# stardist/stardist

Measured on AMD Instinct MI355X. Metric: predict_instances() Mpix/s (2D) + Mvox/s (3D) end-to-end at 1/2/4/8 GPU, higher is better.
Workload: dtype f32

## Files before the change

### stardist_amd/csrc/nms2d.hip

```cpp
#include <type_traits>

#include "common.h"
#include "clip_sweep.h"
#include "clip_beam.h"
#include "area_bounds.h"
#include "poly_pass.h"
#include "nms_rounds.h"
#include "../../include/stardist_hip.h"
#include <hipcub/hipcub.hpp>
#include <math.h>
#include <stdlib.h>
#include <vector>

namespace {

using sdclip::i64;

__device__ __forceinline__ float wave_min(float v) { for (int o = 32; o; o >>= 1) v = fminf(v, __shfl_xor(v, o)); return v; }
__device__ __forceinline__ float wave_max(float v) { for (int o = 32; o; o >>= 1) v = fmaxf(v, __shfl_xor(v, o)); return v; }
__device__ __forceinline__ i64 wave_sum(i64 v) { for (int o = 32; o; o >>= 1) v += __shfl_xor(v, o); return v; }

__global__ void __launch_bounds__(256) k_build(const float* __restrict__ dist, const float* __restrict__ pts,
                                               const float2* __restrict__ sincos, int N, int R,
                                               int* __restrict__ vx, int* __restrict__ vy, int4* __restrict__ bbox,
// ... 67 lines not shown
  if (c < R) ssc[c] = sincos[c];
  {
    const int* g = (const int*)dist + (size_t)base * R;
    const int nv = vec4 ? nel >> 2 : 0;
    for (int e = c; e < nv; e += 64) ((int4*)rows)[e] = ((const int4*)g)[e];
    for (int e = 4 * nv + c; e < nel; e += 64) rows[e] = g[e];
  }
  __syncthreads();
  const bool cv = c < cnt;
  float rmax = 0.f;
  int iy = INT32_MAX, ix = INT32_MAX, iyh = INT32_MIN, ixh = INT32_MIN;
  if (cv) {
    const int i = base + c;
    const float py = pts[2 * i], px = pts[2 * i + 1];
    float xmin = INFINITY, xmax = -INFINITY, ymin = INFINITY, ymax = -INFINITY;
    i64 s = 0, sa = 0;
    int X0 = 0, Y0 = 0, Xp = 0, Yp = 0;
    int k = c % R;
    for (int t = 0; t < R; ++t) {
      const float d = __int_as_float(rows[c * R + k]);
      const float2 sc = ssc[k];
      const float y = py + d * sc.x;
      const float x = px + d * sc.y;
      xmin = fminf(xmin, x); xmax = fmaxf(xmax, x);
      ymin = fminf(ymin, y); ymax = fmaxf(ymax, y);
      rmax = fmaxf(rmax, d);
      const int X = (int)(long long)x, Y = (int)(long long)y;
      sx[c * R + k] = X; sy[c * R + k] = Y;
      if (t) { const i64 cr = (i64)Xp * Y - (i64)Yp * X; s += cr; sa += (cr < 0 ? -cr : cr); }
      else { X0 = X; Y0 = Y; }
      Xp = X; Yp = Y;
      k = (k + 1 == R) ? 0 : k + 1;
    }
    { const i64 cr = (i64)Xp * Y0 - (i64)Yp * X0; s += cr; sa += (cr < 0 ? -cr : cr); }
    float a;
    if (sa < (1ll << 24)) a = (float)s;
    else {
      a = 0.f;
      for (int q = 0; q < R; ++q) {
        const int qn = (q + 1 == R) ? 0 : q + 1;
        a += (float)((i64)sx[c * R + q] * sy[c * R + qn] - (i64)sy[c * R + q] * sx[c * R + qn]);
      }
    }
    area[i] = (float)(0.5 * (double)fabsf(a));
    radius[i] = rmax;
    bbox[i] = make_int4((int)xmin, (int)xmax, (int)ymin, (int)ymax);
    iy = iyh = (int)floorf(py); ix = ixh = (int)floorf(px);
  }
  for (int o = 32; o; o >>= 1) {
    rmax = fmaxf(rmax, __shfl_xor(rmax, o));
    iy = min(iy, __shfl_xor(iy, o)); iyh = max(iyh, __shfl_xor(iyh, o));
    ix = min(ix, __shfl_xor(ix, o)); ixh = max(ixh, __shfl_xor(ixh, o));
  }
  if (c == 0) {
    const int rb = __float_as_int(rmax);
    volatile int* gs = gstats;
    if (rb > gs[0]) atomicMax(&gstats[0], rb);
    if (iy < gs[1]) atomicMin(&gstats[1], iy);
    if (iyh > gs[2]) atomicMax(&gstats[2], iyh);
    if (ix < gs[3]) atomicMin(&gstats[3], ix);
    if (ixh > gs[4]) atomicMax(&gstats[4], ixh);
  }
  __syncthreads();
  {
    int* gx = vx + (size_t)base * R;
    int* gy = vy + (size_t)base * R;
    const int nv = vec4 ? nel >> 2 : 0;
    for (int e = c; e < nv; e += 64) { ((int4*)gx)[e] = ((const int4*)sx)[e]; ((int4*)gy)[e] = ((const int4*)sy)[e]; }
    for (int e = 4 * nv + c; e < nel; e += 64) { gx[e] = sx[e]; gy[e] = sy[e]; }
  }
}

struct GridP { float y0, x0, inv_cs; int ny, nx; };

__device__ __forceinline__ int cell_of(const GridP g, float py, float px, int& cy, int& cx) {
  cy = (int)((py - g.y0) * g.inv_cs); cx = (int)((px - g.x0) * g.inv_cs);
  cy = min(max(cy, 0), g.ny - 1); cx = min(max(cx, 0), g.nx - 1);
  return cy * g.nx + cx;
}

struct Window { int ylo, yhi, xlo, xhi; };
__device__ __forceinline__ Window cell_window(const GridP g, bool by_bbox, float reach, const int4 bb, float py, float px) {
  float y0, y1, x0, x1;
  if (by_bbox) { x0 = (float)bb.x - reach; x1 = (float)bb.y + reach; y0 = (float)bb.z - reach; y1 = (float)bb.w + reach; }
  else { const float rr = 2.f * reach; x0 = px - rr; x1 = px + rr; y0 = py - rr; y1 = py + rr; }
  Window w;
  w.ylo = min(max((int)floorf((y0 - 0.5f - g.y0) * g.inv_cs), 0), g.ny - 1); w.yhi = min(max((int)floorf((y1 + 0.5f - g.y0) * g.inv_cs), 0), g.ny - 1);
  w.xlo = min(max((int)floorf((x0 - 0.5f - g.x0) * g.inv_cs), 0), g.nx - 1); w.xhi = min(max((int)floorf((x1 + 0.5f - g.x0) * g.inv_cs), 0), g.nx - 1);
  return w;
}
constexpr int MAX_WIN_ROWS = 32;

__global__ void k_cell_count(const float* __restrict__ pts, int N, GridP g, int* __restrict__ cellCount, int* __restrict__ candCell) {
  const int i = blockIdx.x * blockDim.x + threadIdx.x;
  if (i >= N) return;
  int cy, cx;
  const int c = cell_of(g, pts[2 * i], pts[2 * i + 1], cy, cx);
  candCell[i] = c;
  atomicAdd(&cellCount[c], 1);
}
struct __attribute__((aligned(16))) CellRec { int4 bb; float py, px, area; int j; };
__global__ void k_cell_fill(int N, const int* __restrict__ candCell, const int* __restrict__ cellStart,
                            int* __restrict__ cellFill, const float* __restrict__ pts, const int4* __restrict__ bbox,
                            const float* __restrict__ area, CellRec* __restrict__ rec, GridP g, int by_bbox, float reach, int* __restrict__ slotCap) {
  const int i = blockIdx.x * blockDim.x + threadIdx.x;
  if (i >= N) return;
  const int c = candCell[i];
  const int pos = atomicAdd(&cellFill[c], 1);
  CellRec r;
  r.bb = bbox[i]; r.py = pts[2 * i]; r.px = pts[2 * i + 1]; r.area = area[i]; r.j = i;
  rec[cellStart[c] + pos] = r;
  if (slotCap) {
    const Window w = cell_window(g, by_bbox != 0, reach, r.bb, r.py, r.px);
    int u = -1;
    for (int yy = w.ylo; yy <= w.yhi; ++yy) u += cellStart[yy * g.nx + w.xhi + 1] - cellStart[yy * g.nx + w.xlo];
    slotCap[i] = u;
    if (i == 0) slotCap[N] = 0;
  }
}

__device__ __forceinline__ bool bbox_intersect(const int4 a, const int4 b) {
  return (b.x <= a.y && a.x <= b.y && b.z <= a.w && a.z <= b.w);
}

__device__ __forceinline__ bool may_interact(const NmsFlags f, const int4 bi, const int4 bj, float pyi, float pxi, float pyj, float pxj,
                                             float ai, float aj) {
  if (f.thr_nonneg) {
    if (!bbox_intersect(bi, bj)) return false;
    const float wh = (float)(min(bi.y, bj.y) - max(bi.x, bj.x)) * (float)(min(bi.w, bj.w) - max(bi.z, bj.z));
    return wh * 1.00001f >= f.thr * fminf(ai, aj) * 0.99999f;
  }
  bool ok = true;
  if (f.use_bbox) ok = ok && bbox_intersect(bi, bj);
  if (f.use_kdtree) {
    const float dy = pyi - pyj, dxx = pxi - pxj;
    const float rr = 2.f * f.max_dist + 1.f;
    ok = ok && (dy * dy + dxx * dxx < rr * rr);
  }
  return ok;
}

struct WindowRuns { int rbeg, excl, nrows, total; };
__device__ __forceinline__ WindowRuns window_runs(const GridP g, const Window win, const int* __restrict__ cellStart, int lane) {
  WindowRuns w;
  w.nrows = __builtin_amdgcn_readfirstlane(win.yhi - win.ylo + 1);
  int rbeg = 0, rlen = 0;
  if (lane < w.nrows) { rbeg = cellStart[(win.ylo + lane) * g.nx + win.xlo]; rlen = cellStart[(win.ylo + lane) * g.nx + win.xhi + 1] - rbeg; }
  int incl = rlen;
  for (int o = 1; o < MAX_WIN_ROWS; o <<= 1) { const int t = __shfl_up(incl, o); if (lane >= o) incl += t; }
  w.total = __builtin_amdgcn_readlane(incl, w.nrows - 1);
  w.rbeg = rbeg; w.excl = incl - rlen;
  return w;
}
template <class Body>
__device__ __forceinline__ void walk_window(const WindowRuns& w, int lane, Body&& body) {
  int r0 = 0;
  for (int t = 0; t < w.total; t += 64) {
    while (r0 + 1 < w.nrows && __builtin_amdgcn_readlane(w.excl, r0 + 1) <= t) ++r0;
    int rb = __builtin_amdgcn_readlane(w.rbeg, r0), re = __builtin_amdgcn_readlane(w.excl, r0);
    const int v = t + lane;
    for (int r = r0 + 1; r < w.nrows; ++r) {
      const int e_r = __builtin_amdgcn_readlane(w.excl, r);
      if (e_r > t + 63) break;
      const int b_r = __builtin_amdgcn_readlane(w.rbeg, r);
      if (e_r <= v) { rb = b_r; re = e_r; }
    }
    body(v < w.total ? rb + (v - re) : -1);
  }
}

template <int MODE>
__global__ void __launch_bounds__(256) k_neighbours(int N, GridP g, NmsFlags f, const CellRec* __restrict__ rec, const int* __restrict__ cellStart,
                                                    int* __restrict__ nbrCount, int* __restrict__ nbrLow, const i64* __restrict__ nbrStart,
                                                    int* __restrict__ nbr, int* __restrict__ waitOn, int by_bbox, float reach) {
  const int wave = threadIdx.x >> 6, lane = threadIdx.x & 63;
  const int per = gridDim.x >> 3;
  const int blk = (blockIdx.x & 7) * per + (blockIdx.x >> 3);
  const int w = blk * (blockDim.x >> 6) + wave;
  if (w >= N) return;
  const CellRec me = rec[w];
  const int i = me.j;
  const int4 bi = me.bb;
  const float pyi = me.py, pxi = me.px, ai = me.area;
  int nLo = 0;
  int minj = INT32_MAX;
  const i64 base = MODE ? nbrStart[i] : 0;
  const WindowRuns runs = window_runs(g, cell_window(g, by_bbox != 0, reach, bi, pyi, pxi), cellStart, lane);
  walk_window(runs, lane, [&](int ri) {
    bool hit = false;
    int j = -1;
    if (ri >= 0) {
      const CellRec r = rec[ri];
      j = r.j;
      if (j < i) hit = may_interact(f, bi, r.bb, pyi, pxi, r.py, r.px, ai, r.area);
    }
    const unsigned long long m = __ballot(hit);
    if (MODE && hit) { nbr[base + nLo + __popcll(m & ((1ull << lane) - 1))] = j; if (j < minj) minj = j; }
    nLo += __popcll(m);
  });
  if (!MODE && lane == 0) nbrCount[i] = nLo;
  if (MODE != 1 && lane == 0) nbrLow[i] = nLo;
  if (MODE) {
    for (int o = 32; o; o >>= 1) minj = min(minj, __shfl_xor(minj, o));
    if (lane == 0) waitOn[i] = (minj < i) ? minj : WAIT_NONE;
  }
}

constexpr int EMIT_STAGE = 512;
__global__ void __launch_bounds__(256) k_round_emit(const int* __restrict__ K, const int* __restrict__ nKPtr, unsigned char* __restrict__ state,
                                                    GridP g, const CellRec* __restrict__ rec, const int* __restrict__ cellStart, int by_bbox, float reach,
                                                    NmsFlags f, const float* __restrict__ pts, const int4* __restrict__ bbox,
                                                    const float* __restrict__ radius, const float* __restrict__ area,
                                                    int2* __restrict__ pairs, unsigned long long* pairCount,
                                                    unsigned long long pairCap) {
  const int wave = threadIdx.x >> 6, lane = threadIdx.x & 63;
  const int nK = *nKPtr;
  __shared__ int2 stage[4][EMIT_STAGE];
  int nst = 0;
  auto flush = [&]() {
    if (!nst) return;
    unsigned long long base = 0;
    if (lane == 0) base = atomicAdd(pairCount, (unsigned long long)nst);
    base = __shfl(base, 0);
    __builtin_amdgcn_wave_barrier();
    for (int k = lane; k < nst; k += 64) { const unsigned long long pos = base + k; if (pos < pairCap) pairs[pos] = stage[wave][k]; }
    __builtin_amdgcn_wave_barrier();
    nst = 0;
  };
  for (int w = blockIdx.x * (blockDim.x >> 6) + wave; w < nK; w += gridDim.x * (blockDim.x >> 6)) {
    const int i = K[w];
    if (lane == 0) state[i] = ST_KEPT;
    const int4 bi = bbox[i];
    const float pyi = pts[2 * i], pxi = pts[2 * i + 1];
    const double ai = (double)area[i] + 1.e-10;
    const float rad = f.max_dist + radius[i];
    const float rad2 = rad * rad;
    const WindowRuns runs = window_runs(g, cell_window(g, by_bbox != 0, reach, bi, pyi, pxi), cellStart, lane);
    walk_window(runs, lane, [&](int ri) {
      bool emit = false;
      int j = -1;
      if (ri >= 0) {
        const CellRec r = rec[ri];
        j = r.j;
        bool ok = j > i;
        if (ok && f.use_kdtree) {
          const float d0 = pyi - r.py, d1 = pxi - r.px;
          float d2 = d0 * d0; d2 += d1 * d1;
          ok = d2 < rad2;
        }
        if (ok && (f.use_bbox || f.thr_nonneg)) {
          const int4 bj = r.bb;
          ok = bbox_intersect(bi, bj);
          if (ok && f.thr_nonneg) {
            const double w = (double)(min(bi.y, bj.y) - max(bi.x, bj.x)), hgt = (double)(min(bi.w, bj.w) - max(bi.z, bj.z));
            const float ub = (float)((w * hgt) / fmin(ai, (double)r.area + 1.e-10));
            if (!(ub > f.thr)) ok = false;
          }
        }
        emit = ok && state[j] == ST_UNDECIDED;
      }
      const unsigned long long m = __ballot(emit);
      if (m) {
        const int c = __popcll(m);
        if (nst + c > EMIT_STAGE) flush();
        if (emit) stage[wave][nst + __popcll(m & ((1ull << lane) - 1))] = make_int2(i, j);
        nst += c;
      }
    });
  }
  flush();
}

template <int MAXV, int S>
__global__ void __launch_bounds__(S) k_prepare(const int* __restrict__ vx, const int* __restrict__ vy, int N, int R,
                                               sdclip::PolyPrep<MAXV>* __restrict__ prep) {
  const int i = blockIdx.x * S + threadIdx.x;
  if (i >= N) return;
  sdclip::PrepWork<sdclip::LdsStorage<S>, MAXV> w;
  w.prepare(vx + (size_t)i * R, vy + (size_t)i * R, R, prep + i);
}

struct PairQueues { unsigned int* spill; unsigned int* spillCount; unsigned int* exact; unsigned int* exactCount; unsigned int cap; };
enum { BEAM_CAPFLAGS = sdclip::ST_OVERFLOW_IL | sdclip::ST_OVERFLOW_REC | sdclip::ST_OVERFLOW_AEL | sdclip::ST_OVERFLOW_LM | sdclip::ST_OVERFLOW_GJ };
template <int MAXV, int K, int MAXIL, int MAXREC, int S, typename CNT, bool REL16 = false>
__global__ void __launch_bounds__(S) k_pairs_beam(const int2* __restrict__ pairs, const unsigned int* __restrict__ idx, const CNT* __restrict__ nPtr,
                                                  const unsigned int* __restrict__ firstPtr, const sdclip::PolyPrep<MAXV>* __restrict__ prep,
                                                  const float* __restrict__ area, float thr, unsigned char* __restrict__ state,
                                                  unsigned char* __restrict__ supp, PairQueues q) {
  typedef typename std::conditional<REL16, sdclip::LdsStorage16<S>, sdclip::LdsStorage<S>>::type Storage;
  typedef sdclip::Beam<MAXV, K, MAXIL, MAXREC, Storage> BeamT;
  const unsigned long long n = (unsigned long long)*nPtr;
  const unsigned long long first = firstPtr ? (unsigned long long)*firstPtr : 0ull;
  const unsigned long long total = n > first ? n - first : 0ull;
  const unsigned long long chunk = (total + gridDim.x - 1) / gridDim.x;
  const bool spread = chunk <= (unsigned long long)S;
  unsigned long long t = spread ? first + (unsigned long long)blockIdx.x * chunk + threadIdx.x : first + (unsigned long long)blockIdx.x * S + threadIdx.x;
  if (spread && (unsigned long long)threadIdx.x >= chunk) t = n;
  const unsigned long long step = spread ? (1ull << 62) : (unsigned long long)gridDim.x * S;
  for (; t < n; t += step) {
    const unsigned int p = idx ? idx[t] : (unsigned int)t;
    const int2 ij = pairs[p];
    BeamT bm;
    bm.reset_state(prep + ij.x, prep + ij.y);
    const i64 twice = bm.execute();
    const int st = bm.status;
    if (st & BEAM_CAPFLAGS) {
      const unsigned int k = atomicAdd(q.spillCount, 1u);
      if (k < q.cap) q.spill[k] = p;
      continue;
    }
    if ((st & ~sdclip::ST_FAIL) || bm.n_joins > 0 || bm.sum_abs_terms >= (1ll << 24)) {
      const unsigned int k = atomicAdd(q.exactCount, 1u);
      if (k < q.cap) q.exact[k] = p;
      continue;
    }
    const float area_inter = 0.5f * (float)twice;
    const float overlap = (float)((double)area_inter / fmin((double)area[ij.x] + 1.e-10, (double)area[ij.y] + 1.e-10));
    if (overlap > thr) { if (supp) supp[p] = 1; else state[ij.y] = ST_SUPPRESSED; }
  }
}
template <int MAXV, int K, int MAXIL, int MAXREC, int S, bool REL16 = false>
size_t beam_lds_bytes() {
  typedef typename std::conditional<REL16, sdclip::LdsStorage16<S>, sdclip::LdsStorage<S>>::type Storage;
  return (size_t)sdclip::Beam<MAXV, K, MAXIL, MAXREC, Storage>::lds_bytes() + 64;
}

__global__ void __launch_bounds__(256) k_pairs_decide(const int2* __restrict__ pairs, const unsigned long long* __restrict__ nPtr,
                                                      const unsigned int* __restrict__ firstPtr, const int* __restrict__ vx, const int* __restrict__ vy, int R,
                                                      const sdarea::PolyProps* __restrict__ props, const float* __restrict__ area, float thr,
                                                      unsigned char* __restrict__ state, unsigned char* __restrict__ supp,
                                                      unsigned char* __restrict__ decided, unsigned int* __restrict__ nDecided) {
  __shared__ float2 sq[4][2][32];
  const int lane = threadIdx.x & 63, half = lane >> 5, l = lane & 31, wv = threadIdx.x >> 6;
  const unsigned long long n = *nPtr, first = firstPtr ? (unsigned long long)*firstPtr : 0ull;
  const unsigned long long nw = (unsigned long long)gridDim.x * 4;
  unsigned int mine = 0;
  for (unsigned long long base = first + 2ull * ((unsigned long long)blockIdx.x * 4 + wv); base < n; base += 2ull * nw) {
    const unsigned long long t = base + half;
    const bool active = t < n;
    const int2 ij = active ? pairs[t] : make_int2(0, 0);
    const sdarea::PolyProps pp = props[ij.x], pq = props[ij.y];
    const sdarea::Enclosure E = sdarea::pair_enclosure(vx + (size_t)ij.x * R, vy + (size_t)ij.x * R, vx + (size_t)ij.y * R, vy + (size_t)ij.y * R, R, pp, pq,
                                                       active, sq[wv][half], l, half);
    if (active && l == 0) {
      const int dec = sdarea::decide(E, area[ij.x], area[ij.y], thr);
      decided[t] = (unsigned char)dec;
      if (dec == 2) { if (supp) supp[t] = 1; else state[ij.y] = ST_SUPPRESSED; }
      if (dec) ++mine;
    }
    __builtin_amdgcn_wave_barrier();
  }
  mine += __shfl_xor(mine, 32);
  if (lane == 0 && mine) atomicAdd(nDecided, mine);
}

__global__ void __launch_bounds__(256) k_tail_emit(const int* __restrict__ U, int nU, const unsigned char* __restrict__ state,
                                                   const i64* __restrict__ nbrStart, const int* __restrict__ nbrLow, const int* __restrict__ nbr, NmsFlags f,
                                                   const float* __restrict__ pts, const int4* __restrict__ bbox,
                                                   const float* __restrict__ radius, const float* __restrict__ area,
                                                   int2* __restrict__ pairs, unsigned long long* pairCount, unsigned long long pairCap,
                                                   unsigned int* __restrict__ segStart, int* __restrict__ segCnt) {
  const int wave = threadIdx.x >> 6, lane = threadIdx.x & 63;
  for (int w = blockIdx.x * (blockDim.x >> 6) + wave; w < nU; w += gridDim.x * (blockDim.x >> 6)) {
    const int j = U[w];
    int cnt = 0;
    unsigned long long base = 0;
    if (state[j] == ST_UNDECIDED) {
      const i64 beg = nbrStart[j], end = beg + nbrLow[j];
      const int4 bj = bbox[j];
      const float pyj = pts[2 * j], pxj = pts[2 * j + 1];
      const float aj = area[j];
      for (int pass = 0; pass < 2; ++pass) {
        int k = 0;
        for (i64 t = beg; t < end; t += 64) {
          const i64 id = t + lane;
          bool emit = false;
          int i = -1;
          if (id < end) {
            i = nbr[id];
            if (i < j && state[i] == ST_UNDECIDED) {
              bool ok = true;
              if (f.use_kdtree) {
                const float rad = f.max_dist + radius[i];
                const float d0 = pts[2 * i] - pyj, d1 = pts[2 * i + 1] - pxj;
                float d2 = d0 * d0; d2 += d1 * d1;
                ok = d2 < rad * rad;
              }
              if (ok && (f.use_bbox || f.thr_nonneg)) {
                const int4 bi = bbox[i];
                ok = bbox_intersect(bi, bj);
                if (ok && f.thr_nonneg) {
                  const double w2 = (double)(min(bi.y, bj.y) - max(bi.x, bj.x)), hgt = (double)(min(bi.w, bj.w) - max(bi.z, bj.z));
                  const float ub = (float)((w2 * hgt) / fmin((double)area[i] + 1.e-10, (double)aj + 1.e-10));
                  if (!(ub > f.thr)) ok = false;
                }
              }
              emit = ok;
            }
          }
          const unsigned long long m = __ballot(emit);
          if (pass == 1 && emit) {
            const unsigned long long pos = base + k + __popcll(m & ((1ull << lane) - 1));
            if (pos < pairCap) pairs[pos] = make_int2(i, j);
          }
          k += __popcll(m);
        }
        if (pass == 0) {
          cnt = k;
// ... 205 lines not shown
  static int prepare(const int* vx, const int* vy, int N, int R, void* prep, hipStream_t s) {
    if constexpr (MAXV == 32) {
      if (sdpass::launch_poly_pass(vx, vy, N, R, nullptr, prep, s)) { sd::set_error("sd_nms2d: launch of the per-polygon pass failed"); return -1; }
      return 0;
    } else {
      const size_t lds = sdclip::PrepWork<sdclip::LdsStorage<SPREP>, MAXV>::lds_bytes() + 64;
      hipLaunchKernelGGL((k_prepare<MAXV, SPREP>), dim3(sd::div_up(N, SPREP)), dim3(SPREP), lds, s, vx, vy, N, R, (Prep*)prep);
      SD_LAUNCH_CHECK();
      return 0;
    }
  }
  static int tier1(const int2* pairs, const unsigned int* idx, const unsigned long long* nPairs, const unsigned int* first, const void* prep, const float* area,
                   float thr, unsigned char* state, unsigned char* supp, PairQueues q, hipStream_t s) {
    const int lanes = sd::option(sd::OPT_NMS2D_PAIR_LANES);
    if (lanes == 32) {
      static const size_t lds32 = beam_lds_bytes<MAXV, 8, 6, 4, 32>();
      hipLaunchKernelGGL((k_pairs_beam<MAXV, 8, 6, 4, 32, unsigned long long>), dim3(256 * 8), dim3(32), lds32, s, pairs, idx, nPairs, first, (const Prep*)prep, area, thr, state, supp, q);
    } else if (lanes == 6464) {
      static const size_t lds = beam_lds_bytes<MAXV, 8, 6, 4, 64>();
      hipLaunchKernelGGL((k_pairs_beam<MAXV, 8, 6, 4, 64, unsigned long long>), dim3(256 * 4), dim3(64), lds, s, pairs, idx, nPairs, first, (const Prep*)prep, area, thr, state, supp, q);
    } else {
      static const size_t lds16 = beam_lds_bytes<MAXV, 8, 6, 4, 64, true>();
      static const int per_cu = (int)((160 * 1024) / lds16);
      hipLaunchKernelGGL((k_pairs_beam<MAXV, 8, 6, 4, 64, unsigned long long, true>), dim3(256 * per_cu), dim3(64), lds16, s, pairs, idx, nPairs, first, (const Prep*)prep, area, thr, state, supp, q);
    }
    SD_LAUNCH_CHECK();
    return 0;
  }
  template <typename CNT>
  static int tier2(const int2* pairs, const unsigned int* idx, const CNT* nPairs, const unsigned int* first, const void* prep, const float* area, float thr,
                   unsigned char* state, unsigned char* supp, PairQueues q, hipStream_t s) {
    static const size_t lds = beam_lds_bytes<MAXV, 15, 16, 8, 32>();
    hipLaunchKernelGGL((k_pairs_beam<MAXV, 15, 16, 8, 32, CNT>), dim3(256 * 3), dim3(32), lds, s, pairs, idx, nPairs, first, (const Prep*)prep, area, thr, state, supp, q);
    SD_LAUNCH_CHECK();
    return 0;
  }
};
}

namespace {
int launch_build(sd::Arena& A, hipStream_t s, const float* d_dist, const float* d_points, int N, int R, int* vx, int* vy, int4* bbox,
                 float* radius, float* area, int** gstatsOut, hipEvent_t evStart) {
  const int gs_init[8] = {0, INT32_MAX, INT32_MIN, INT32_MAX, INT32_MIN, 0, 0, 0};
  std::vector<float> hdr(8 + 2 * (size_t)R);
  memcpy(hdr.data(), gs_init, sizeof(gs_init));
  const float ANGLE_PI = 2 * M_PI / R;
  for (int k = 0; k < R; ++k) { hdr[8 + 2 * k] = sinf(ANGLE_PI * k); hdr[8 + 2 * k + 1] = cosf(ANGLE_PI * k); }
  int* gstats = A.take_n<int>(8 + 2 * (size_t)R);
  if (!gstats) return -1;
  const float2* d_sc = (const float2*)(gstats + 8);
  SD_CHECK(hipMemcpyAsync(gstats, hdr.data(), hdr.size() * sizeof(float), hipMemcpyHostToDevice, s));
  if (evStart) SD_CHECK(hipEventRecord(evStart, s));
  if (R <= 32) {
    const int vec4 = ((((uintptr_t)d_dist | (uintptr_t)vx | (uintptr_t)vy) & 15) == 0) ? 1 : 0;
    hipLaunchKernelGGL(k_build32, dim3(sd::div_up(N, 64)), dim3(64), 2 * 64 * (size_t)R * sizeof(int), s, d_dist, d_points, d_sc, N, R, vec4,
                       vx, vy, bbox, radius, area, gstats);
  } else
    hipLaunchKernelGGL(k_build, dim3(sd::div_up(N, 4)), dim3(256), 4 * 2 * R * sizeof(int), s, d_dist, d_points, d_sc, N, R,
                       vx, vy, bbox, radius, area, gstats);
  SD_LAUNCH_CHECK();
  *gstatsOut = gstats;
  return 0;
}
}

extern "C" int sd_nms2d_build_device(const float* d_dist, const float* d_points, int n_polys, int n_rays, int32_t* d_vx, int32_t* d_vy,
                                     int32_t* d_bbox, float* d_radius, float* d_area, int32_t* d_gstats, void* stream_) {
  hipStream_t s = (hipStream_t)stream_;
  if (n_polys <= 0) return 0;
  if (n_rays < 1 || n_rays > 256) { sd::set_error("sd_nms2d_build: n_rays=%d unsupported (1..256)", n_rays); return -1; }
  sd::Arena& A = sd::arena();
  if (A.begin(s)) return -1;
  int* gstats = nullptr;
  if (launch_build(A, s, d_dist, d_points, n_polys, n_rays, d_vx, d_vy, (int4*)d_bbox, d_radius, d_area, &gstats, nullptr)) return -1;
  SD_CHECK(hipMemcpyAsync(d_gstats, gstats, 5 * sizeof(int), hipMemcpyDeviceToDevice, s));
  SD_CHECK(hipStreamSynchronize(s));
  return 0;
}

extern "C" int sd_nms2d_device(const float* d_dist, const float* d_points, int n_polys, int n_rays, int use_kdtree,
                               int use_bbox, int verbose, float threshold, uint8_t* d_keep, int64_t* stats,
                               void* stream_) {
  hipStream_t s = (hipStream_t)stream_;
  const int N = n_polys, R = n_rays;
  if (stats) memset(stats, 0, 16 * sizeof(int64_t));
  if (N <= 0) return 0;
  if (R < 1 || R > 256) { sd::set_error("sd_nms2d: n_rays=%d unsupported (1..256)", R); return -1; }
  if (verbose) {
    printf("Non Maximum Suppression (2D) ++++ \n");
    printf("NMS: n_polys    = %d \nNMS: n_rays     = %d  \nNMS: thresh     = %.3f \nNMS: use_bbox   = %d\nNMS: use_kdtree = %d\n",
           N, R, threshold, use_bbox, use_kdtree);
    printf("NMS: using HIP (gfx950), uniform-grid broad phase + scan-beam pair kernel\n");
  }
  sd::Arena& A = sd::arena();
  if (A.begin(s)) return -1;
  hipEvent_t ev0 = nullptr, ev1 = nullptr;
  if (stats) { SD_CHECK(hipEventCreate(&ev0)); SD_CHECK(hipEventCreate(&ev1)); }
  struct EvGuard { hipEvent_t a, b; ~EvGuard() { if (a) (void)hipEventDestroy(a); if (b) (void)hipEventDestroy(b); } } evguard{ev0, ev1};
  double ns_pairs = 0, ns_full = 0, ns_pre = 0;
  long long n_pair_launches = 0;

  if (!use_kdtree && !use_bbox && threshold < 0) {
    SD_CHECK(hipMemsetAsync(d_keep, 0, N, s));
    SD_CHECK(hipMemsetAsync(d_keep, 1, 1, s));
    SD_CHECK(hipStreamSynchronize(s));
    return 0;
  }

  int* vx = A.take_n<int>((size_t)N * R);
  int* vy = A.take_n<int>((size_t)N * R);
  int4* bbox = A.take_n<int4>(N);
  float* radius = A.take_n<float>(N);
  float* area = A.take_n<float>(N);
  unsigned char* state = A.take_n<unsigned char>(N);
  int* candCell = A.take_n<int>(N);
  int* gstats = nullptr;
  if (!vx || !vy || !bbox || !radius || !area || !state || !candCell) return -1;
  if (launch_build(A, s, d_dist, d_points, N, R, vx, vy, bbox, radius, area, &gstats, stats ? ev0 : nullptr)) return -1;
  size_t prepStride;
  if (R <= 32) prepStride = sizeof(sdclip::PolyPrep<32>); else if (R <= 64) prepStride = sizeof(sdclip::PolyPrep<64>);
  else if (R <= 128) prepStride = sizeof(sdclip::PolyPrep<128>); else prepStride = sizeof(sdclip::PolyPrep<256>);
  void* prep = A.take((size_t)N * prepStride);
  if (!prep) return -1;
  hipStream_t side = sd::side_stream();
  if (!side) return -1;
  hipEvent_t evFork = nullptr, evJoin = nullptr;
  SD_CHECK(hipEventCreateWithFlags(&evFork, hipEventDisableTiming));
  SD_CHECK(hipEventCreateWithFlags(&evJoin, hipEventDisableTiming));
  EvGuard evguardFJ{evFork, evJoin};
  const bool areaBounds = R <= 32 && R >= 3 && sd::option(sd::OPT_NMS2D_AREA_BOUNDS) != 0 && sd::option(sd::OPT_NMS2D_STRICT) == 0;
  sdarea::PolyProps* props = nullptr;
  hipEvent_t evProps = nullptr, evPrep = nullptr;
  SD_CHECK(hipEventCreateWithFlags(&evProps, hipEventDisableTiming));
  SD_CHECK(hipEventCreateWithFlags(&evPrep, hipEventDisableTiming));
  EvGuard evguardP{evProps, evPrep};
  if (areaBounds) {
    props = (sdarea::PolyProps*)A.take((size_t)N * sizeof(sdarea::PolyProps));
    if (!props) return -1;
  }
  auto launch_side = [&]() -> int {
    SD_CHECK(hipEventRecord(evFork, s));
    SD_CHECK(hipStreamWaitEvent(side, evFork, 0));
    int rc;
    if (R <= 32) rc = sdpass::launch_poly_pass(vx, vy, N, R, props, prep, side);
    else if (R <= 64) rc = BeamPath<64, 64>::prepare(vx, vy, N, R, prep, side);
    else if (R <= 128) rc = BeamPath<128, 32>::prepare(vx, vy, N, R, prep, side);
    else rc = BeamPath<256, 16>::prepare(vx, vy, N, R, prep, side);
    if (rc) { sd::set_error("sd_nms2d: launch of the per-polygon pass failed"); return -1; }
    SD_CHECK(hipEventRecord(evProps, side));
    SD_CHECK(hipEventRecord(evPrep, side));
    SD_CHECK(hipEventRecord(evJoin, side));
    return 0;
  };
  int gs[8];
  SD_CHECK(hipMemcpyAsync(gs, gstats, sizeof(gs), hipMemcpyDeviceToHost, s));
  SD_CHECK(hipStreamSynchronize(s));
  float max_dist;
  memcpy(&max_dist, &gs[0], 4);

  GridP g;
  const float reach = (max_dist + 1.f) * 1.0001f + 1e-3f;
  const int by_bbox = (threshold >= 0.f || use_bbox) ? 1 : 0;
  float cs = 0.5f * reach;
  if (!(cs >= 1.f)) cs = 1.f;
  for (;;) {
    g.ny = (int)(((double)gs[2] - gs[1]) / cs) + 1;
    g.nx = (int)(((double)gs[4] - gs[3]) / cs) + 1;
    if ((long long)g.ny * g.nx <= (1ll << 26)) break;
    cs *= 2.f;
  }
  g.y0 = (float)gs[1]; g.x0 = (float)gs[3]; g.inv_cs = 1.f / cs;
  const int nCells = g.ny * g.nx;
  int* cellCount = A.take_n<int>(2 * ((size_t)nCells + 1));
  int* cellFill = cellCount ? cellCount + nCells + 1 : nullptr;
  int* cellStart = A.take_n<int>(nCells + 1);
  CellRec* cellRec = (CellRec*)A.take((size_t)N * sizeof(CellRec));
  int* nbrCount = A.take_n<int>(N + 1);
  i64* nbrStart = A.take_n<i64>(N + 1);
  int* nbrLow = A.take_n<int>(N + 1);
  if (!cellCount || !cellStart || !cellFill || !cellRec || !nbrCount || !nbrStart || !nbrLow) return -1;
  SD_CHECK(hipMemsetAsync(cellCount, 0, 2 * ((size_t)nCells + 1) * sizeof(int), s));
  hipLaunchKernelGGL(k_cell_count, dim3(sd::div_up(N, 256)), dim3(256), 0, s, d_points, N, g, cellCount, candCell);
  SD_LAUNCH_CHECK();
  size_t tmpBytes = 0, tmpBytes2 = 0;
  (void)hipcub::DeviceScan::ExclusiveSum(nullptr, tmpBytes, cellCount, cellStart, nCells + 1, s);
  (void)hipcub::DeviceScan::ExclusiveSum(nullptr, tmpBytes2, nbrCount, nbrStart, N + 1, s);
  if (tmpBytes2 > tmpBytes) tmpBytes = tmpBytes2;
  void* scanTmp = A.take(tmpBytes + 256);
  if (!scanTmp) return -1;
  SD_CHECK(hipcub::DeviceScan::ExclusiveSum(scanTmp, tmpBytes, cellCount, cellStart, nCells + 1, s));
  const bool singlePass = sd::option(sd::OPT_NMS2D_NBR_SINGLE) != 0;
  hipLaunchKernelGGL(k_cell_fill, dim3(sd::div_up(N, 256)), dim3(256), 0, s, N, candCell, cellStart, cellFill, d_points, bbox, area, cellRec, g, by_bbox, reach,
                     singlePass ? nbrCount : (int*)nullptr);
  SD_LAUNCH_CHECK();
  int* U0 = A.take_n<int>(N);
  unsigned char* pend0 = A.take_n<unsigned char>(N);
  int* head0 = A.take_n<int>(N);
  unsigned int* dcount0 = A.take_n<unsigned int>(1);
  if (!U0 || !pend0 || !head0 || !dcount0) return -1;
  hipLaunchKernelGGL(k_round_lists_init, dim3(sd::div_up(N, 256)), dim3(256), 0, s, N, U0, state, pend0, head0, dcount0);

  NmsFlags f;
  f.use_kdtree = use_kdtree; f.use_bbox = use_bbox; f.thr_nonneg = (threshold >= 0.f); f.thr = threshold; f.max_dist = max_dist;

  const int nbBlocks = (sd::div_up(N, 4) + 7) & ~7;
  NbrLists L{};
  L.count = nbrCount; L.low = nbrLow; L.start = nbrStart; L.lowOnly = true;
  auto launch_neighbours = [&](int mode, const NbrLists& l) {
    if (mode == 0)
      hipLaunchKernelGGL((k_neighbours<0>), dim3(nbBlocks), dim3(256), 0, s, N, g, f, cellRec, cellStart, nbrCount, nbrLow, (const i64*)nullptr, (int*)nullptr,
                         (int*)nullptr, by_bbox, reach);
    else if (mode == 1)
      hipLaunchKernelGGL((k_neighbours<1>), dim3(nbBlocks), dim3(256), 0, s, N, g, f, cellRec, cellStart, nbrCount, nbrLow, (const i64*)nbrStart, l.nbr, l.waitOn, by_bbox, reach);
    else
      hipLaunchKernelGGL((k_neighbours<2>), dim3(nbBlocks), dim3(256), 0, s, N, g, f, cellRec, cellStart, nbrCount, nbrLow, (const i64*)nbrStart, l.nbr, l.waitOn, by_bbox, reach);
  };
  const int rcLists = build_neighbour_lists(A, s, N, singlePass, scanTmp, tmpBytes, launch_neighbours, launch_side, L);
  if (rcLists > 0) {
    sd::set_error("sd_nms2d: %lld neighbour entries for %d candidates exceed the capacity of one call (2^31 - 1): shard the input "
                  "(predict_instances_sharded / predict_instances_big)", (long long)L.total, N);
    return -1;
  }
  if (rcLists) return -1;
  const int* nbr = L.nbr;
  int* waitOn = L.waitOn;
  const i64 totalNbr = 2 * L.total;

  SD_CHECK(hipStreamWaitEvent(s, evProps, 0));
  if (stats) { SD_CHECK(hipEventRecord(ev1, s)); SD_CHECK(hipEventSynchronize(ev1)); float ms = 0; SD_CHECK(hipEventElapsedTime(&ms, ev0, ev1)); ns_pre = ms * 1e6; }

  const unsigned long long pairCap = (unsigned long long)(totalNbr / 2 + 64);
  int* U1 = A.take_n<int>(N);
  int* K = A.take_n<int>(N);
  int2* pairs = A.take_n<int2>(pairCap);
  const unsigned int qCap = (unsigned int)(pairCap < (1ull << 30) ? pairCap : (1ull << 30));
  unsigned int* spillPairs = A.take_n<unsigned int>(qCap);
  unsigned int* exactPairs = A.take_n<unsigned int>(qCap);
  int* Sl = A.take_n<int>(N);
  Counters* d_cnt = (Counters*)A.take(sizeof(Counters));
  static const bool pairSort = sd::tuning_env("SD_NMS_PAIR_SORT", 1) != 0;
  unsigned int* pairOrder = pairSort && R <= 32 ? A.take_n<unsigned int>(qCap) : nullptr;
  unsigned int* bucketHist = A.take_n<unsigned int>(2 * PAIR_BUCKETS);
  unsigned long long* nOrdered = A.take_n<unsigned long long>(1);
  if (!U0 || !U1 || !K || !pairs || !spillPairs || !exactPairs || !Sl || !d_cnt || !bucketHist || !nOrdered || (pairSort && R <= 32 && !pairOrder)) return -1;
  unsigned char* decided = (areaBounds && pairOrder) ? A.take_n<unsigned char>(pairCap) : nullptr;
  if (areaBounds && pairOrder && !decided) return -1;
  i64 totalDecided = 0, totalSkipped = 0;
  int nU = N, rounds = 0;
  i64 totalPairs = 0, totalExact = 0, totalSpill = 0;
  int* Ucur = U0; int* Unext = U1;
  Counters h;
  hipEvent_t ev2 = nullptr, ev3 = nullptr;
  if (stats) { SD_CHECK(hipEventCreate(&ev2)); SD_CHECK(hipEventCreate(&ev3)); }
  EvGuard evguard2{ev2, ev3};
  static const int tailDiv = sd::tuning_env("SD_NMS_TAIL_DIV", 6);
  static const int tailMax = sd::tuning_env("SD_NMS_TAIL_MAX", 65536);
  const int tailT = tailDiv > 0 ? ((N / tailDiv) < tailMax ? (N / tailDiv) : tailMax) : -1;
  unsigned char* supp = nullptr; unsigned int* segStart = nullptr; int* segCnt = nullptr;
  static const bool deferEnv = sd::tuning_env("SD_NMS_DEFER", 1) != 0;
  const bool deferOn = tailT >= 0 && deferEnv;
  Deferred dfr{nullptr, nullptr, nullptr, nullptr, nullptr, qCap};
  unsigned int* firstNew = A.take_n<unsigned int>(1);
  dfr.pend = pend0; dfr.head = head0; dfr.count = dcount0;
  if (!firstNew) return -1;
  if (deferOn) {
    dfr.pairs = A.take_n<int2>(qCap);
    dfr.next = A.take_n<int>(qCap);
    if (!dfr.pairs || !dfr.next) return -1;
  }
  i64 nDeferred = 0;
  bool sideGeneral = false;
  unsigned int* nNewExact = A.take_n<unsigned int>(1);
  if (!nNewExact) return -1;
  const int deferFrom = (deferOn && decided) ? sd::option(sd::OPT_NMS2D_DEFER_UNDECIDED) : 0;
  const unsigned int deferMax = (unsigned int)(sd::option(sd::OPT_NMS2D_DEFER_MAX) > 0 ? sd::option(sd::OPT_NMS2D_DEFER_MAX) : 0);
  unsigned char* defKind = nullptr; unsigned int* nJoinDef = nullptr;
  if (deferFrom > 0) {
    defKind = A.take_n<unsigned char>(qCap); nJoinDef = A.take_n<unsigned int>(1);
    if (!defKind || !nJoinDef) return -1;
    SD_CHECK(hipMemsetAsync(defKind, 0, qCap, s));
  }
  i64 totalUndecDeferred = 0;
  i64 nUndecDeferredUpper = 0;
  auto run_pairs = [&](unsigned char* suppOut) -> int {
    const unsigned int* first = suppOut ? firstNew : nullptr;
    if (stats) SD_CHECK(hipEventRecord(ev0, s));
    PairQueues q1{spillPairs, &d_cnt->nSpill, exactPairs, &d_cnt->nExact, qCap};
    PairQueues q2{exactPairs, &d_cnt->nExact, exactPairs, &d_cnt->nExact, qCap};
    int rc;
    if (R <= 32) {
      if (pairOrder) {
        static const int keyMode = sd::tuning_env("SD_NMS_PAIR_KEY", 2);
        static const int modes[6][3] = {{1, 32, 32}, {1, 64, 16}, {1, 64, 64}, {16, 16, 16}, {16, 32, 8}, {4, 32, 32}};
        const int* md = modes[keyMode >= 0 && keyMode < 6 ? keyMode : 2];
        const PairKey key{(const char*)prep, prepStride, 1.f / (4.f * (max_dist + 1.f)), md[0], md[1], md[2]};
        SD_CHECK(hipMemsetAsync(bucketHist, 0, PAIR_BUCKETS * sizeof(unsigned int), s));
        if (decided)
          hipLaunchKernelGGL(k_pairs_decide, dim3(256 * 8), dim3(256), 0, s, pairs, &d_cnt->nPairs, first, vx, vy, R, props, area, threshold, state, suppOut,
                             decided, &d_cnt->nDecided);
        if (!suppOut && deferFrom > 0 && rounds >= deferFrom)
          hipLaunchKernelGGL(k_defer_undecided, dim3(256), dim3(256), 0, s, pairs, &d_cnt->nPairs, &d_cnt->nDecided, deferMax, decided, state, dfr, defKind, &d_cnt->nErr);
        const unsigned int* bfirst = (suppOut && deferFrom > 0) ? nullptr : first;
        SD_CHECK(hipStreamWaitEvent(s, evPrep, 0));
        const unsigned char* liveState = suppOut ? nullptr : state;
        hipLaunchKernelGGL(k_pair_bucket_count, dim3(512), dim3(256), 0, s, pairs, &d_cnt->nPairs, bfirst, d_points, key, bucketHist, decided, liveState,
                           &d_cnt->nSkipped);
        hipLaunchKernelGGL(k_pair_bucket_scan, dim3(1), dim3(1024), 0, s, bucketHist, bucketHist + PAIR_BUCKETS, nOrdered);
        hipLaunchKernelGGL(k_pair_bucket_scatter, dim3(512), dim3(256), 0, s, pairs, &d_cnt->nPairs, bfirst, d_points, key, bucketHist + PAIR_BUCKETS,
                           pairOrder, qCap, decided, liveState);
        SD_LAUNCH_CHECK();
        rc = BeamPath<32, 64>::tier1(pairs, pairOrder, nOrdered, (const unsigned int*)nullptr, prep, area, threshold, state, suppOut, q1, s);
      } else {
        SD_CHECK(hipStreamWaitEvent(s, evPrep, 0));
        rc = BeamPath<32, 64>::tier1(pairs, (const unsigned int*)nullptr, &d_cnt->nPairs, first, prep, area, threshold, state, suppOut, q1, s);
      }
      if (stats) SD_CHECK(hipEventRecord(ev1, s));
      if (!rc) rc = BeamPath<32, 64>::tier2(pairs, spillPairs, &d_cnt->nSpill, (const unsigned int*)nullptr, prep, area, threshold, state, suppOut, q2, s);
    } else {
      SD_CHECK(hipStreamWaitEvent(s, evPrep, 0));
      if (R <= 64) rc = BeamPath<64, 64>::tier2(pairs, (const unsigned int*)nullptr, &d_cnt->nPairs, first, prep, area, threshold, state, suppOut, q2, s);
      else if (R <= 128) rc = BeamPath<128, 32>::tier2(pairs, (const unsigned int*)nullptr, &d_cnt->nPairs, first, prep, area, threshold, state, suppOut, q2, s);
      else rc = BeamPath<256, 16>::tier2(pairs, (const unsigned int*)nullptr, &d_cnt->nPairs, first, prep, area, threshold, state, suppOut, q2, s);
      if (stats) SD_CHECK(hipEventRecord(ev1, s));
    }
    if (rc) return -1;
    if (stats) SD_CHECK(hipEventRecord(ev2, s));
    if (!suppOut && deferOn) {
      hipLaunchKernelGGL(k_defer, dim3(64), dim3(256), 0, s, pairs, exactPairs, &d_cnt->nExact, qCap, dfr, &d_cnt->nErr);
      SD_LAUNCH_CHECK();
    } else if (suppOut && sideGeneral) {
      hipLaunchKernelGGL(k_count_after, dim3(1), dim3(1), 0, s, nNewExact, &d_cnt->nExact, deferFrom > 0 ? nJoinDef : firstNew);
      SD_LAUNCH_CHECK();
      if (sd::clip_full_pairs(pairs, exactPairs + nDeferred, nNewExact, qCap - (unsigned int)nDeferred, R, vx, vy, area, threshold, state, suppOut, &d_cnt->nErr, s)) return -1;
      SD_CHECK(hipStreamWaitEvent(s, evJoin, 0));
    } else if (sd::clip_full_pairs(pairs, exactPairs, &d_cnt->nExact, qCap, R, vx, vy, area, threshold, state, suppOut, &d_cnt->nErr, s)) return -1;
    if (stats) SD_CHECK(hipEventRecord(ev3, s));
    return 0;
  };
  auto account = [&](const char* what) -> int {
    if (h.nPairs > pairCap || h.nSpill > qCap || h.nExact > qCap) { sd::set_error("sd_nms2d: pair queue overflow (internal error)"); return -1; }
    if (h.nErr) { sd::set_error("sd_nms2d: %u pairs exceeded the general path's fixed capacities or the deferred-pair list (with more than 64 rays: at least that many; the launch stops at the first)", h.nErr); return -1; }
    totalPairs += (i64)h.nPairs; totalExact += h.nExact; totalSpill += h.nSpill; totalDecided += h.nDecided; totalSkipped += h.nSkipped;
    if (stats) {
      float ms = 0, ms2 = 0;
      SD_CHECK(hipEventElapsedTime(&ms, ev0, ev1)); SD_CHECK(hipEventElapsedTime(&ms2, ev2, ev3));
      if (h.nPairs) { ns_pairs += ms * 1e6; ++n_pair_launches; }
      ns_full += ms2 * 1e6;
      if (sd::option(sd::OPT_TRACE)) printf("%s %d: nU=%d nK=%d pairs=%llu decided by the area enclosure=%u j already suppressed=%u spill=%u exact=%u pair_kernel=%.3f ms general_path=%.3f ms\n", what, rounds, h.nU, h.nK, h.nPairs, h.nDecided, h.nSkipped, h.nSpill, h.nExact, ms, ms2);
    }
    return 0;
  };
  bool forceTail = false;
  while (nU > 0) {
    ++rounds;
    if (tailT >= 0 && ((nU <= tailT && rounds > 1) || forceTail)) {
      if (!supp) { supp = A.take_n<unsigned char>(pairCap); segStart = A.take_n<unsigned int>(N); segCnt = A.take_n<int>(N); }
      if (!supp || !segStart || !segCnt) return -1;
      SD_CHECK(hipMemsetAsync(d_cnt, 0, sizeof(Counters), s));
      SD_CHECK(hipMemsetAsync(supp, 0, pairCap, s));
      const int wg = sd::div_up(nU, 4) < 2048 ? sd::div_up(nU, 4) : 2048;
      if (deferFrom > 0) {
        hipLaunchKernelGGL(k_tail_init2, dim3(64), dim3(256), 0, s, dfr, defKind, pairs, exactPairs, &d_cnt->nPairs, &d_cnt->nExact, firstNew, decided, state,
                           &d_cnt->nSkipped);
        hipLaunchKernelGGL(k_copy_u32, dim3(1), dim3(1), 0, s, nJoinDef, &d_cnt->nExact);
      } else
        hipLaunchKernelGGL(k_tail_init, dim3(64), dim3(256), 0, s, dfr, pairs, exactPairs, &d_cnt->nPairs, &d_cnt->nExact, firstNew);
      sideGeneral = deferOn && nDeferred > 0 && nDeferred < (i64)qCap && side != nullptr;
      if (sideGeneral) {
        SD_CHECK(hipEventRecord(evFork, s));
        SD_CHECK(hipStreamWaitEvent(side, evFork, 0));
        if (sd::clip_full_pairs(pairs, exactPairs, deferFrom > 0 ? nJoinDef : firstNew, qCap, R, vx, vy, area, threshold, state, supp, &d_cnt->nErr, side)) return -1;
        SD_CHECK(hipEventRecord(evJoin, side));
      }
      hipLaunchKernelGGL(k_tail_emit, dim3(wg), dim3(256), 0, s, Ucur, nU, state, nbrStart, nbrLow, nbr, f, d_points, bbox, radius, area, pairs,
                         &d_cnt->nPairs, pairCap, segStart, segCnt);
      SD_LAUNCH_CHECK();
      if (run_pairs(supp)) return -1;
      hipEvent_t evr0 = nullptr, evr1 = nullptr;
      const bool tr = stats && sd::option(sd::OPT_TRACE);
      if (tr) { SD_CHECK(hipEventCreate(&evr0)); SD_CHECK(hipEventCreate(&evr1)); SD_CHECK(hipEventRecord(evr0, s)); }
      for (int it = 0; it < 10; ++it)
// ... 263 lines not shown
```

Before: 316.2.

## Prefetch cell records in NMS window walk and launch side pass earlier

Window walking in the 2D NMS neighbour and emit kernels now software-pipelines the cell-record loads. It keeps WALK_DEPTH 64-entry batches of records in flight as raw int4 pairs, so global-load latency overlaps with the interaction tests. Separately, the side-stream polygon property pass is launched before the host sync on grid stats rather than inside neighbour-list construction. A scope guard drains the side stream on early error return. This costs extra registers per wave, and invalid lanes issue redundant loads of record 0.

```diff
diff --git a/stardist_amd/csrc/nms2d.hip b/stardist_amd/csrc/nms2d.hip
--- a/stardist_amd/csrc/nms2d.hip
+++ b/stardist_amd/csrc/nms2d.hip
@@ -243,20 +243,43 @@
   w.rbeg = rbeg; w.excl = incl - rlen;
   return w;
 }
+__device__ __forceinline__ int step_index(const WindowRuns& w, int lane, int t, int& r0) {
+  while (r0 + 1 < w.nrows && __builtin_amdgcn_readlane(w.excl, r0 + 1) <= t) ++r0;
+  int rb = __builtin_amdgcn_readlane(w.rbeg, r0), re = __builtin_amdgcn_readlane(w.excl, r0);
+  const int v = min(t + lane, w.total - 1);
+  for (int r = r0 + 1; r < w.nrows; ++r) {
+    const int e_r = __builtin_amdgcn_readlane(w.excl, r);
+    if (e_r > t + 63) break;
+    const int b_r = __builtin_amdgcn_readlane(w.rbeg, r);
+    if (e_r <= v) { rb = b_r; re = e_r; }
+  }
+  return rb + (v - re);
+}
+struct RecRegs { int4 lo, hi; };
+__device__ __forceinline__ RecRegs load_rec(const CellRec* __restrict__ rec, int ri) {
+  const int4* p = (const int4*)(rec + ri);
+  RecRegs r; r.lo = p[0]; r.hi = p[1];
+  return r;
+}
+#ifndef SD_NMS2D_WALK_DEPTH
+#define SD_NMS2D_WALK_DEPTH 3
+#endif
+constexpr int WALK_DEPTH = SD_NMS2D_WALK_DEPTH;
 template <class Body>
-__device__ __forceinline__ void walk_window(const WindowRuns& w, int lane, Body&& body) {
+__device__ __forceinline__ void walk_window(const WindowRuns& w, const CellRec* __restrict__ rec, int lane, Body&& body) {
   int r0 = 0;
-  for (int t = 0; t < w.total; t += 64) {
-    while (r0 + 1 < w.nrows && __builtin_amdgcn_readlane(w.excl, r0 + 1) <= t) ++r0;
-    int rb = __builtin_amdgcn_readlane(w.rbeg, r0), re = __builtin_amdgcn_readlane(w.excl, r0);
-    const int v = t + lane;
-    for (int r = r0 + 1; r < w.nrows; ++r) {
-      const int e_r = __builtin_amdgcn_readlane(w.excl, r);
-      if (e_r > t + 63) break;
-      const int b_r = __builtin_amdgcn_readlane(w.rbeg, r);
-      if (e_r <= v) { rb = b_r; re = e_r; }
-    }
-    body(v < w.total ? rb + (v - re) : -1);
+  auto fetch = [&](int t) { return load_rec(rec, t < w.total ? step_index(w, lane, t, r0) : 0); };
+  RecRegs q[WALK_DEPTH];
+#pragma unroll
+  for (int d = 0; d < WALK_DEPTH; ++d) q[d] = fetch(64 * d);
+  for (int t = 0; t < w.total; t += 64 * WALK_DEPTH) {
+#pragma unroll
+    for (int d = 0; d < WALK_DEPTH; ++d) {
+      const int ts = t + 64 * d;
+      if (ts >= w.total) break;
+      body(q[d], ts + lane < w.total);
+      q[d] = fetch(ts + 64 * WALK_DEPTH);
+    }
   }
 }
 
@@ -277,14 +300,10 @@
   int minj = INT32_MAX;
   const i64 base = MODE ? nbrStart[i] : 0;
   const WindowRuns runs = window_runs(g, cell_window(g, by_bbox != 0, reach, bi, pyi, pxi), cellStart, lane);
-  walk_window(runs, lane, [&](int ri) {
-    bool hit = false;
-    int j = -1;
-    if (ri >= 0) {
-      const CellRec r = rec[ri];
-      j = r.j;
-      if (j < i) hit = may_interact(f, bi, r.bb, pyi, pxi, r.py, r.px, ai, r.area);
-    }
+  walk_window(runs, rec, lane, [&](const RecRegs& r, bool valid) {
+    const int j = r.hi.w;
+    const bool hit = valid && j < i &&
+                     may_interact(f, bi, r.lo, pyi, pxi, __int_as_float(r.hi.x), __int_as_float(r.hi.y), ai, __int_as_float(r.hi.z));
     const unsigned long long m = __ballot(hit);
     if (MODE && hit) { nbr[base + nLo + __popcll(m & ((1ull << lane) - 1))] = j; if (j < minj) minj = j; }
     nLo += __popcll(m);
@@ -327,24 +346,22 @@
     const float rad = f.max_dist + radius[i];
     const float rad2 = rad * rad;
     const WindowRuns runs = window_runs(g, cell_window(g, by_bbox != 0, reach, bi, pyi, pxi), cellStart, lane);
-    walk_window(runs, lane, [&](int ri) {
+    walk_window(runs, rec, lane, [&](const RecRegs& r, bool valid) {
       bool emit = false;
-      int j = -1;
-      if (ri >= 0) {
-        const CellRec r = rec[ri];
-        j = r.j;
-        bool ok = j > i;
+      const int j = r.hi.w;
+      {
+        bool ok = valid && j > i;
         if (ok && f.use_kdtree) {
-          const float d0 = pyi - r.py, d1 = pxi - r.px;
+          const float d0 = pyi - __int_as_float(r.hi.x), d1 = pxi - __int_as_float(r.hi.y);
           float d2 = d0 * d0; d2 += d1 * d1;
           ok = d2 < rad2;
         }
         if (ok && (f.use_bbox || f.thr_nonneg)) {
-          const int4 bj = r.bb;
+          const int4 bj = r.lo;
           ok = bbox_intersect(bi, bj);
           if (ok && f.thr_nonneg) {
             const double w = (double)(min(bi.y, bj.y) - max(bi.x, bj.x)), hgt = (double)(min(bi.w, bj.w) - max(bi.z, bj.z));
-            const float ub = (float)((w * hgt) / fmin(ai, (double)r.area + 1.e-10));
+            const float ub = (float)((w * hgt) / fmin(ai, (double)__int_as_float(r.hi.z) + 1.e-10));
             if (!(ub > f.thr)) ok = false;
           }
         }
@@ -856,6 +873,12 @@
     SD_CHECK(hipEventRecord(evJoin, side));
     return 0;
   };
+  const bool sideEarly = sd::tuning_env("SD_NMS_SIDE_EARLY", 1) != 0;
+  bool sideLaunched = false;
+  auto side_once = [&]() -> int { if (sideLaunched) return 0; sideLaunched = true; return launch_side(); };
+  struct SideDrain { hipStream_t st; const bool* launched; bool armed; ~SideDrain() { if (armed && *launched) (void)hipStreamSynchronize(st); } }
+      sideDrain{side, &sideLaunched, true};
+  if (sideEarly && side_once()) return -1;
   int gs[8];
   SD_CHECK(hipMemcpyAsync(gs, gstats, sizeof(gs), hipMemcpyDeviceToHost, s));
   SD_CHECK(hipStreamSynchronize(s));
@@ -919,7 +942,7 @@
     else
       hipLaunchKernelGGL((k_neighbours<2>), dim3(nbBlocks), dim3(256), 0, s, N, g, f, cellRec, cellStart, nbrCount, nbrLow, (const i64*)nbrStart, l.nbr, l.waitOn, by_bbox, reach);
   };
-  const int rcLists = build_neighbour_lists(A, s, N, singlePass, scanTmp, tmpBytes, launch_neighbours, launch_side, L);
+  const int rcLists = build_neighbour_lists(A, s, N, singlePass, scanTmp, tmpBytes, launch_neighbours, side_once, L);
   if (rcLists > 0) {
     sd::set_error("sd_nms2d: %lld neighbour entries for %d candidates exceed the capacity of one call (2^31 - 1): shard the input "
                   "(predict_instances_sharded / predict_instances_big)", (long long)L.total, N);
@@ -931,6 +954,7 @@
   const i64 totalNbr = 2 * L.total;
 
   SD_CHECK(hipStreamWaitEvent(s, evProps, 0));
+  sideDrain.armed = false;
   if (stats) { SD_CHECK(hipEventRecord(ev1, s)); SD_CHECK(hipEventSynchronize(ev1)); float ms = 0; SD_CHECK(hipEventElapsedTime(&ms, ev0, ev1)); ns_pre = ms * 1e6; }
 
   const unsigned long long pairCap = (unsigned long long)(totalNbr / 2 + 64);
```

Result: no change. 321.0, median of 6 (+1.5%).
